# keb721/mc_water_ls_mw

Measured on AMD Instinct MI355X. Metric: mW interactions/sec/GPU (full-box + single-move ΔE), 4096-mol ice; 1/2/4/8-GPU replica scaling, higher is better.
Workload: dtype f64; 1 GPU; ih4096_t015: 4096-molecule ice-Ih boxes (8x8x8 x 8-atom cell, sigma 0.15 A), per step: full-box energy of every walker + old/new local energy of every trial move; walkers_per_gpu=512, moves_per_walker=2048, molecules=4096, parallelism=replica farm: 1 x 512 independent walkers, one process per GPU, exchange=one nccl all-reduce of 3 x 101 f64 per step (one-rank process group)

## Files before the change

### include/mw_energy.h

```cpp
#ifndef MW_ENERGY_H
#define MW_ENERGY_H

#include <stdint.h>

#ifdef __cplusplus
extern "C" {
#endif

#define MW_MAXNEIGH_LIMIT 64
#define MW_MAX_IVECT      1024

#define MW_DISPATCH_BUILD    0
#define MW_DISPATCH_ENERGY   1
#define MW_DISPATCH_MOVES    2
#define MW_DISPATCH_FORCES   3
#define MW_DISPATCH_ICE      4
#define MW_DISPATCH_RDF      5
#define MW_DISPATCH_FAMILIES 6
#define MW_DISPATCH_FIELDS   13

#define MW_LDS_ENERGY 0
#define MW_LDS_FORCES 1
#define MW_LDS_ICE    2
#define MW_LDS_MOVE   3
#define MW_LDS_SORT   4
#define MW_LDS_ORDER  5
#define MW_LDS_BUILDS 6


int mw_init(int device, int nwater, int nboxes, int maxneigh);
int mw_finalize(void);
int mw_is_initialised(void);

const char *mw_last_error(void);

int mw_constants(double out[8]);


int mw_set_cell(int ils, const double h[9], int *nivect_out);
int mw_set_cells_range(int first_ils, int count, const double *h, int *nivect_out);
int mw_get_ivects(int ils, double *out, int max_vectors, int *nivect_out);

int mw_upload_positions(int ils, const double *xyz);
int mw_download_positions(int ils, double *xyz);
int mw_upload_positions_range(int first_ils, int count, const double *xyz);
int mw_download_positions_range(int first_ils, int count, double *xyz);
int mw_patch_position(int ils, int imol, const double r[3]);


int mw_build_neighbours(int ils, int *min_nn, int *max_nn);
int mw_build_neighbours_batch(int first_ils, int count, int *min_nn, int *max_nn);
int mw_get_neighbours(int ils, int *nn, int *jn, int *vn);


int mw_model_energy(int ils, double *e);
int mw_model_energy_of(int ils, const double *xyz, double *e);
int mw_model_energy_batch(int first_ils, int count, double *e_out);
int mw_model_energy_counts(int ils, long long *npairs, long long *ntriplets);
int mw_model_energy_counts_total(int first_ils, int count, long long *npairs, long long *ntriplets);
int mw_neighbour_total(int first_ils, int count, long long *total_entries);


int mw_model_forces(int ils, double *e, double *f, double *w);
int mw_model_forces_batch(int first_ils, int count, double *e, double *f, double *w);
int mw_model_forces_launch(int first_ils, int count, int timer_slot);


int mw_ice_classes(int ils, double rc, uint8_t *cls, int counts[6]);
int mw_ice_classes_batch(int first_ils, int count, double rc, uint8_t *cls, int *counts);
int mw_ice_classes_launch(int first_ils, int count, double rc, int timer_slot);
int mw_ice_bonds(int ils, double rc, double *c);

// ... 92 lines not shown
```

### mc_water_ls_mw_amd/csrc/mw_host_ctx.hip.h

```cpp
#pragma once

namespace {

thread_local std::string g_err;
std::recursive_mutex g_mu;
std::shared_mutex g_gate;
int g_depth = 0;
struct DeviceGuard;
struct ExclusiveGuard;
#define MW_LOCK ExclusiveGuard mw_lock_; DeviceGuard mw_dev_; if (mw_lock_.rc) return 1

int fail(const char* fmt, ...)
{
    char buf[512];
    va_list ap;
    va_start(ap, fmt);
    vsnprintf(buf, sizeof buf, fmt, ap);
    va_end(ap);
    g_err = buf;
    return 1;
}

#define HIPCHK(call)                                                                             \
    do {                                                                                         \
// ... 87 lines not shown
    size_t tabscratch_n = 0;
    unsigned long long* d_wvol = nullptr;
    int* d_wflag = nullptr;
    double* d_wwin = nullptr;
    double *d_wfac = nullptr, *d_wsum = nullptr;
    int* d_winflag = nullptr;
    double* d_wmom = nullptr; size_t wmom_cap = 0;
    double* d_wstep = nullptr;
    bool has_steps = false;
    int sweep_log_ahead = 8;
    bool has_windows = false;
    int* d_wls = nullptr;
    double* d_wmu = nullptr;
    unsigned long long* d_wacc = nullptr;
    double* d_swlog = nullptr;
    size_t swlog_cap = 0;
    hipStream_t sstream = nullptr;
    mw::MailHead* h_head = nullptr;  mw::MailHead* d_head = nullptr;
    mw::MailSlot* h_slots = nullptr; mw::MailSlot* d_slots = nullptr;
    mw::MailSlot* req_slots = nullptr;
    mw::MailSlot* d_req = nullptr;
    void* req_dev_alloc = nullptr;
    int nslots = 0;
    bool srv_running = false, srv_enabled = true;
    unsigned long long sseq[8] = {0, 0, 0, 0, 0, 0, 0, 0};
    unsigned long long spend[8] = {0, 0, 0, 0, 0, 0, 0, 0};
    unsigned long long spend_epoch[8] = {0, 0, 0, 0, 0, 0, 0, 0};
    int spend_box[8] = {0, 0, 0, 0, 0, 0, 0, 0};
    hipEvent_t ev_srv = nullptr;
    double* d_pm = nullptr; int* d_srvmomok = nullptr;
    int* d_srvunc = nullptr;
    unsigned long long* d_srvcounts = nullptr;
    long long srv_starts = 0;
    int mcap = 0, mn = 0;
    int* d_mimol = nullptr;
    double *d_mtrial = nullptr, *d_meold = nullptr, *d_menew = nullptr;
    unsigned int* d_mcnt = nullptr;
    unsigned int* d_mtot = nullptr; int mtot_cap = 0, mtot_n = 0;
    int* d_mperm = nullptr;
    int* d_mdecl = nullptr;
    int mdecl_par = 0;
    int4* d_mwork = nullptr;
    int mwork_cap = 0, mwork_n = 0;
    bool mlds = false;
    int mmode = 0;
    int m_boxlo = 0, m_boxhi = -1, m_minreq = 0;
    enum { kCountsThere = 0, kCountsPending = 1, kCountsDropped = 2 };
    int mcnt_state = kCountsThere;
    int mcnt_passes = 0;
    bool move_sort = true;
    bool move_masks = true;
    bool move_gate = true;
    bool move_pairs32 = true;
    bool move_counts_eager = false;
    int move_moments = -1;
    int mchunk = 16;
    bool m_noself = false;
};

Ctx g;
std::mutex g_slot_mu[8];
std::mutex g_srv_mu;
std::atomic<unsigned long long> g_epoch{0};
std::atomic<bool> g_srv_enabled{true};

int server_stop();

struct ExclusiveGuard {
    int rc = 0;
    ExclusiveGuard()
    {
        g_mu.lock();
        if (g_depth++ == 0) {
            g_gate.lock(); g_epoch.fetch_add(1, std::memory_order_relaxed);
            g.mom_count = 0;
            if (g.srv_running) rc = server_stop();
            if (g.live && g.h_slots)
                for (int sl = 0; sl < g.nslots && sl < 8; ++sl)
                    if (g.spend[sl] && reinterpret_cast<volatile unsigned long long*>(&g.h_slots[sl].rep_seq)[0] != g.spend[sl]) {
                        reinterpret_cast<volatile unsigned long long*>(&g.h_slots[sl].rep_seq)[0] = g.spend[sl];
                        std::atomic_thread_fence(std::memory_order_seq_cst);
                    }
        }
    }
    ~ExclusiveGuard()
    {
        if (--g_depth == 0) g_gate.unlock();
        g_mu.unlock();
    }
};

struct DeviceGuard {
    int prev = -1;
    bool switched = false;
    DeviceGuard()
    {
        if (g.live && hipGetDevice(&prev) == hipSuccess && prev != g.device)
            switched = hipSetDevice(g.device) == hipSuccess;
    }
    ~DeviceGuard() { if (switched) (void)hipSetDevice(prev); }
};

constexpr size_t kQueue1024 = (size_t)(mw::kQCap + 1) * 1024 * sizeof(uint32_t);
constexpr size_t kQueue256 = (size_t)(mw::kQCap + 1) * 256 * sizeof(uint32_t);
constexpr int kFullLayout = mw::kLayoutPair;
size_t model_lds_bytes(int N, int ivcap) { return kQueue1024 + mw::lds_vec_bytes((size_t)N) + mw::lds_vec_bytes((size_t)ivcap); }
bool lds_fits(int N, int ivcap)
{
    return model_lds_bytes(N, ivcap) <= (size_t)kLdsBudget;
}
size_t pos_lds_bytes(int N, int ivcap) { return mw::lds_vec_bytes((size_t)N) + mw::lds_vec_bytes((size_t)ivcap); }
constexpr size_t kMoveScratch = 16 * sizeof(mw::WaveScratch);
size_t move_lds_bytes(int N, int ivcap, int chunk)
{
    return kMoveScratch + mw::lds_vec_bytes((size_t)ivcap) + mw::lds_vec_bytes((size_t)N) + (((size_t)N + 7) & ~(size_t)7) + (size_t)chunk * sizeof(int);
}
static_assert((size_t)kLdsBudget / 25 < ((size_t)1 << mw::kKeyMolBits), "a staged box's molecules fit the key of mw_move_energy.hip.h");
bool lds_fits_move(int N, int ivcap)
{
    return move_lds_bytes(N, ivcap, mw::kMoveChunk) <= (size_t)kLdsBudget;
}
int cell_stride(int N) { return N + 64; }
size_t sort_lds_bytes(int N) { return (size_t)N * 24 + ((size_t)cell_stride(N) + 1) * 4; }
bool sort_fits(int N) { return N <= mw::kSortBoxMax; }
void order_plan(int N, int seg_override, int& seg, int& kbits)
{
    seg = lds_fits(N, 32) ? ((N + 63) & ~63) : 64;
    if (seg_override >= 64) seg = (seg_override + 63) & ~63;
    const size_t seg_groups = ((size_t)std::min(N, seg) + 63) / 64;
    kbits = -1;
    for (int kb = 8; kb >= 0; --kb)
        if ((seg_groups << kb) <= (size_t)mw::kOrderSlots) { kbits = kb; break; }
}
size_t order_lds_bytes(int N, int seg, int kbits)
{
    return kbits < 0 ? 0 : sizeof(int) * ((((size_t)std::min(N, seg) + 63) / 64) << kbits);
}

int check_live() { return g.live ? 0 : fail("mw: engine not initialised (call mw_init / energy_init first)"); }
int check_box(int ils) { return (ils >= 1 && ils <= g.nbox) ? 0 : fail("mw: box index %d outside 1..%d", ils, g.nbox); }
int check_range(int first, int count)
{
    return (first >= 1 && count >= 1 && first + count - 1 <= g.nbox)
               ? 0 : fail("mw: box range %d..%d outside 1..%d", first, first + count - 1, g.nbox);
}
int check_mol(int imol) { return (imol >= 1 && imol <= g.N) ? 0 : fail("mw: molecule index %d outside 1..%d", imol, g.N); }
enum Form { kLaunch, kBatch, kSingle };
int check_boxes(int first, int count, Form form) { return form == kSingle ? check_box(first) : check_range(first, count); }

void drop_move_counts() { if (g.mcnt_state == Ctx::kCountsPending) g.mcnt_state = Ctx::kCountsDropped; }
void drop_driver_moments(bool state_changed = true) { g.swm_count = 0; if (state_changed) drop_move_counts(); }

int dev_free_bytes(void** p)
{
    if (!*p) return 0;
    g.owned.erase(std::remove(g.owned.begin(), g.owned.end(), *p), g.owned.end());
    void* q = *p;
    *p = nullptr;
    HIPCHK(hipFree(q));
    return 0;
}
int dev_alloc_bytes(void** p, size_t bytes)
{
    if (*p) {
        HIPCHK(hipStreamSynchronize(g.stream));
        if (dev_free_bytes(p)) return 1;
    }
    HIPCHK(hipMalloc(p, bytes));
    g.owned.push_back(*p);
// ... 67 lines not shown
```

### mc_water_ls_mw_amd/csrc/mw_host_moves.hip.h

```cpp
#pragma once

namespace {

int ensure_moves(int n)
{
    if (n <= g.mcap) return 0;
    size_t cap = 1024;
    while (cap < (size_t)n) cap *= 2;
    g.mcap = 0;
    if (dev_alloc(g.d_mimol, cap) || dev_alloc(g.d_mtrial, 3 * cap) || dev_alloc(g.d_meold, cap) || dev_alloc(g.d_menew, cap) ||
        dev_alloc(g.d_mcnt, 4 * cap) || dev_alloc(g.d_mperm, cap) || dev_alloc(g.d_mdecl, 2 * cap + 2)) return 1;
    HIPCHK(hipMemset(g.d_mdecl, 0, 2 * sizeof(int)));
    g.mdecl_par = 0;
    g.mcap = (int)cap;
    return 0;
}

template <typename Kernel>
void launch_move_kernel(Kernel kernel, size_t shmem, int kmode, const double* mom, unsigned int* tot)
{
    hipLaunchKernelGGL(kernel, dim3(g.mwork_n), dim3(1024), shmem, g.stream,
                       g.d_pos, g.d_ivect, g.d_nivect, g.d_listm, g.d_nn, g.d_mwork, g.d_mimol, g.d_mtrial, g.d_mperm,
                       g.d_meold, g.d_menew, g.d_mcnt, g.d_mdecl, g.N, g.ivcap, kmode, mom, tot);
}

}

extern "C" {

int mw_moves_upload(int n, const int* ils, const int* imol, const double* trial_xyz)
{
    MW_LOCK;
    if (check_live()) return 1;
    if (n < 0) return fail("mw_moves_upload: n = %d", n);
    drop_move_counts();
    g.mn = 0;
    if (n == 0) return 0;
    if (!ils || !imol) return fail("mw_moves_upload: null request arrays");
    std::vector<int> cnt((size_t)g.nbox + 1, 0);
    for (int m = 0; m < n; ++m) {
        if (ils[m] < 1 || ils[m] > g.nbox) return fail("mw_moves_upload: request %d has box %d outside 1..%d", m, ils[m], g.nbox);
        if (imol[m] < 1 || imol[m] > g.N) return fail("mw_moves_upload: request %d has molecule %d outside 1..%d", m, imol[m], g.N);
        ++cnt[(size_t)ils[m]];
    }
    std::vector<int> start((size_t)g.nbox + 1, 0);
    int used_boxes = 0;
    g.m_noself = true;
    g.m_boxlo = g.nbox; g.m_boxhi = -1; g.m_minreq = n;
    for (int b = 0; b < g.nbox; ++b) {
        start[(size_t)b + 1] = start[b] + cnt[(size_t)b + 1];
        if (cnt[(size_t)b + 1]) {
            ++used_boxes; if (!g.h_usegrid[(size_t)b]) g.m_noself = false;
            g.m_boxlo = std::min(g.m_boxlo, b); g.m_boxhi = std::max(g.m_boxhi, b); g.m_minreq = std::min(g.m_minreq, cnt[(size_t)b + 1]);
        }
    }
    std::vector<int> perm((size_t)n), i0((size_t)n), fill(start.begin(), start.end() - 1);
    std::vector<double> tr(trial_xyz ? (size_t)3 * n : 0);
    for (int m = 0; m < n; ++m) {
        const int s = fill[(size_t)ils[m] - 1]++;
        perm[s] = m; i0[s] = imol[m] - 1;
        if (trial_xyz) { tr[3 * (size_t)s] = trial_xyz[3 * (size_t)m]; tr[3 * (size_t)s + 1] = trial_xyz[3 * (size_t)m + 1]; tr[3 * (size_t)s + 2] = trial_xyz[3 * (size_t)m + 2]; }
    }
    g.mlds = lds_fits_move(g.N, g.ivcap) && ((long long)n * 2048 >= (long long)used_boxes * 24 * g.N);
    int chunk = 16;
    if (g.mlds) {
        const long long want = (long long)n / (2LL * std::max(1, g.cu));
        chunk = 256;
        while (chunk < mw::kMoveChunk && chunk < want) chunk *= 2;
        if (const char* ev = std::getenv("MW_MOVE_CHUNK")) { const int v = std::atoi(ev); if (v >= 64 && v <= mw::kMoveChunk) chunk = v; }
    }
    g.mchunk = chunk;
    { const char* ms = std::getenv("MW_MOVE_SORT"); g.move_sort = !(ms && ms[0] == '0'); }
    { const char* mk = std::getenv("MW_MOVE_MASKS"); g.move_masks = !(mk && mk[0] == '0'); }
    { const char* mg = std::getenv("MW_MOVE_GATE"); g.move_gate = !(mg && mg[0] == '0'); }
    { const char* mp = std::getenv("MW_MOVE_PAIRS32"); g.move_pairs32 = !(mp && mp[0] == '0'); }
    std::vector<int4> work;
    for (int b = 0; b < g.nbox; ++b) {
        const int s0 = start[b], cntb = start[(size_t)b + 1] - s0;
        if (cntb == 0) continue;
        const int nitems = (cntb + chunk - 1) / chunk;
        for (int k = 0; k < nitems; ++k) {
            int4 w; w.x = b; w.y = s0 + (int)((long long)cntb * k / nitems); w.z = s0 + (int)((long long)cntb * (k + 1) / nitems); w.w = 0;
            work.push_back(w);
        }
    }
    if (getenv("MW_NO_XCD_ORDER") == nullptr && work.size() >= 16) {
        constexpr int kXcd = 8;
        std::vector<std::vector<int4>> seq(kXcd);
        int boxrank = -1, lastbox = -1;
        for (const int4& w : work) {
            if (w.x != lastbox) { ++boxrank; lastbox = w.x; }
            seq[(size_t)(boxrank % kXcd)].push_back(w);
        }
        std::vector<int4> ordered;
        ordered.reserve(work.size());
        std::vector<size_t> at(kXcd, 0);
        while (ordered.size() < work.size())
            for (int x = 0; x < kXcd; ++x)
                if (at[x] < seq[x].size()) ordered.push_back(seq[x][at[x]++]);
        work.swap(ordered);
    }
    if (ensure_moves(n)) return 1;
    if (dev_grow(g.d_mwork, g.mwork_cap, work.size(), 2 * work.size())) return 1;
    HIPCHK(hipMemcpyAsync(g.d_mwork, work.data(), sizeof(int4) * work.size(), hipMemcpyHostToDevice, g.stream));
    HIPCHK(hipMemcpyAsync(g.d_mperm, perm.data(), sizeof(int) * n, hipMemcpyHostToDevice, g.stream));
    HIPCHK(hipMemcpyAsync(g.d_mimol, i0.data(), sizeof(int) * n, hipMemcpyHostToDevice, g.stream));
    if (trial_xyz) HIPCHK(hipMemcpyAsync(g.d_mtrial, tr.data(), sizeof(double) * 3 * n, hipMemcpyHostToDevice, g.stream));
    HIPCHK(hipStreamSynchronize(g.stream));
    g.mwork_n = (int)work.size();
    g.mn = n;
    return 0;
}

static int launch_moves(int mode)
{
    if (g.mn == 0) return 0;
    g.mcnt_state = Ctx::kCountsDropped;
    if (dev_grow(g.d_mtot, g.mtot_cap, (size_t)g.mwork_n, 2 * (size_t)g.mwork_n, 4)) return 1;
    g.mtot_n = 0;
    const size_t iv_bytes = kMoveScratch + mw::lds_vec_bytes((size_t)g.ivcap);
    const int kmode = mode | (g.mdecl_par << 2);
    g.mdecl_par ^= 1;
    const bool mom_ok = g.mlds && g.m_noself && model_geo(1).lds && g.m_boxhi >= g.m_boxlo;
    const bool fresh = g.d_mom && g.mom_count > 0 && g.mom_first - 1 <= g.m_boxlo && g.m_boxhi < g.mom_first - 1 + g.mom_count;
    const bool use_mom = mom_ok && (g.move_moments >= 0 ? g.move_moments != 0 : g.m_minreq >= (fresh ? 512 : 1280));
    const size_t shmem = g.mlds ? move_lds_bytes(g.N, g.ivcap, g.mchunk) : iv_bytes;
    auto launch = [&](auto kernel, const double* mom, unsigned int* tot, int bits = 0) { launch_move_kernel(kernel, shmem, kmode | bits, mom, tot); };
    if (use_mom) {
        if (!fresh && launch_model_energy(g.m_boxlo + 1, g.m_boxhi - g.m_boxlo + 1, true, false)) return 1;
        launch(mw::k_move_energy<true, mw::kLayoutSoA, false, true>, g.d_mom, g.d_mtot, (g.move_counts_eager ? 8 : 0) | (g.move_sort ? 32 : 0) | (g.move_masks ? 64 : 0) | (g.move_gate ? 128 : 0) | (g.move_pairs32 ? 256 : 0));
        if (g.move_counts_eager) g.mtot_n = g.mwork_n;
    } else if (g.mlds && g.m_noself) launch(mw::k_move_energy<true, mw::kLayoutSoA, false>, nullptr, nullptr);
    else if (g.mlds)                 launch(mw::k_move_energy<true>, nullptr, nullptr);
    else                             launch(mw::k_move_energy<false>, nullptr, nullptr);
    HIPCHK(hipGetLastError());
    g.mcnt_state = use_mom && !g.move_counts_eager ? Ctx::kCountsPending : Ctx::kCountsThere;
    {
        int* d = g.disp[MW_DISPATCH_MOVES];
        d[0] = g.ivcap; d[1] = g.mn; d[2] = g.mlds; d[3] = g.m_noself; d[4] = use_mom; d[5] = use_mom && fresh; d[6] = g.mchunk;
        d[7] = g.mwork_n; d[8] = (int)shmem; d[9] = use_mom ? 3 : (g.mlds ? (g.m_noself ? 2 : 1) : 0);
        d[10] = g.mcnt_state; d[11] = g.mcnt_passes; d[12] = -1;
    }
    hipLaunchKernelGGL(mw::k_move_fallback, dim3(std::min(1024, (g.mn + 3) / 4)), dim3(256), 0, g.stream, g.d_pos, g.d_ivect, g.d_listm, g.d_nn,
                       g.d_mimol, g.d_mtrial, g.d_mperm, g.d_meold, g.d_menew, g.d_mcnt, g.d_mdecl, g.N, g.ivcap, kmode);
    HIPCHK(hipGetLastError());
    g.mmode = mode;
    return 0;
}

int mw_moves_launch(void)
{
    MW_LOCK;
    if (check_live()) return 1;
    return launch_moves(3);
}

int mw_step_launch(int first_ils, int count, int timer_slot)
{
    MW_LOCK;
    if (check_live() || check_range(first_ils, count)) return 1;
    Timers t;
    if (t.open("mw_step_launch", timer_slot, 2) || t.start(0)) return 1;
    const bool want_mom = g.mn > 0 && g.mlds && g.m_noself && (g.move_moments >= 0 ? g.move_moments != 0 : g.m_minreq >= 512);
    if (launch_model_energy(first_ils, count, want_mom, true)) return 1;
    if (t.stop(0) || t.start(1) || launch_moves(3)) return 1;
    return t.stop(1);
}

int mw_moves_fetch(double* e_old, double* e_new)
{
    MW_LOCK;
    if (check_live()) return 1;
    if (g.mn > 0) {
        if (e_old) HIPCHK(hipMemcpyAsync(e_old, g.d_meold, sizeof(double) * g.mn, hipMemcpyDeviceToHost, g.stream));
        if (e_new) HIPCHK(hipMemcpyAsync(e_new, g.d_menew, sizeof(double) * g.mn, hipMemcpyDeviceToHost, g.stream));
    }
    HIPCHK(hipStreamSynchronize(g.stream));
    return 0;
}

int mw_moves_counts(long long out[4])
{
    MW_LOCK;
    if (check_live()) return 1;
    out[0] = out[1] = out[2] = out[3] = 0;
    if (g.mn == 0) return 0;
    if (g.mcnt_state == Ctx::kCountsDropped)
        return fail("mw_moves_counts: the counts of the last launch were not made, and the launch failed or the requests, positions, cells "
                    "or lists it saw have changed since: ask right after a launch (or run with MW_MOVE_COUNTS=eager)");
    if (g.mcnt_state == Ctx::kCountsPending) {
        launch_move_kernel(mw::k_move_energy<true, mw::kLayoutSoA, false, true>, move_lds_bytes(g.N, g.ivcap, g.mchunk), g.mmode | 8 | 16 | (g.move_sort ? 32 : 0) | (g.move_masks ? 64 : 0) | (g.move_gate ? 128 : 0) | (g.move_pairs32 ? 256 : 0), g.d_mom, g.d_mtot);
        HIPCHK(hipGetLastError());
        g.mtot_n = g.mwork_n;
        g.mcnt_state = Ctx::kCountsThere;
// ... 40 lines not shown
```

### mc_water_ls_mw_amd/csrc/mw_move_energy.hip.h

```cpp
#pragma once
#include <type_traits>

#include "mw_common.hip.h"
#include "mw_local_energy.hip.h"
#include "mw_move_scan.hip.h"
#include "mw_move_moments.hip.h"
#include "mw_move_lanes.hip.h"

namespace mw {

constexpr int kMoveChunk = 2048;

constexpr int kKeyMolBits = 13, kKeyReqBits = 11, kKeyNqBits = 5;
constexpr int kKeyReqShift = kKeyMolBits, kKeyNqShift = kKeyMolBits + kKeyReqBits;
constexpr uint32_t kKeyMolMask = (1u << kKeyMolBits) - 1u, kKeyReqMask = (1u << kKeyReqBits) - 1u;
constexpr int kKeyNqOver = kLaneQueue + 1;
constexpr int kSortBins = kKeyNqOver + 1;
constexpr int kSortChunks = kMoveChunk / 64;
static_assert(kMoveChunk <= (1 << kKeyReqBits) && kKeyNqOver < (1 << kKeyNqBits) && kKeyNqShift + kKeyNqBits <= 32, "the key's fields");
static_assert(kSortChunks == 2 * 16, "two rounds of the sixteen wavefronts rank an item's keys: chunks v and v + 16 in wavefront v");
static_assert((kSortChunks + 1) * kSortBins * sizeof(uint32_t) <= 16 * sizeof(WaveScratch), "the sort's tables are overlaid on the idle queues");
constexpr size_t kQueueBytes = kLaneQueueWords * sizeof(uint32_t);
constexpr size_t kMaskTableAt = 16 * kQueueBytes;
static_assert(kMaskTableAt + kMoveChunk * sizeof(uint32_t) <= 16 * sizeof(WaveScratch), "the queues and the mask table fit the scratch blocks: no new LDS");
static_assert((kSortChunks + 1) * kSortBins * sizeof(uint32_t) <= kMaskTableAt, "the sort's tables lie on the queues and end before the masks");
static_assert(kMaskTableAt % 16 == 0 && kQueueBytes % 16 == 0, "alignment of the queues and of the mask table");

template <bool LDSPOS, int LAYOUT = kLayoutSoA, bool SELFIMG = true, bool MOMPATH = false>
__global__ __launch_bounds__(1024)
void k_move_energy(const double* __restrict__ pos, const double* __restrict__ ivect,
                   const int* __restrict__ nivect, const uint32_t* __restrict__ listm,
                   const int* __restrict__ nn, const int4* __restrict__ work,
                   const int* __restrict__ req_imol, const double* __restrict__ req_trial,
                   const int* __restrict__ perm,
                   double* __restrict__ e_old, double* __restrict__ e_new,
                   unsigned int* __restrict__ counts,
                   int* __restrict__ declined,
                   int N, int ivcap, int mode, const double* __restrict__ mom = nullptr,
                   unsigned int* __restrict__ mtot = nullptr)
{
    static_assert(!MOMPATH || (LDSPOS && !SELFIMG), "the moment path serves boxes staged in LDS whose cells hold no self-images");
    __shared__ unsigned char s_qn[MOMPATH ? kCap * (kCap - 1) : 2];
    unsigned int acc[4] = {0u, 0u, 0u, 0u};
    extern __shared__ __attribute__((aligned(16))) double smem[];
    const int4 w = work[blockIdx.x];
    const int b = w.x;
    const int tid = threadIdx.x, lane = tid & 63, wave = tid >> 6;
    const bool count = !MOMPATH || (mode & 8) != 0, quiet = MOMPATH && (mode & 16) != 0;
    const double* P  = pos + (size_t)b * N * 3;
    const double* IV = ivect + (size_t)b * ivcap * 3;
    const uint32_t* LM = listm + (size_t)b * N * kRow;
    const int* NN = nn + (size_t)b * N;
    const int niv = nivect[b];

    double* spos = smem;
    double* siv = smem + (LDSPOS ? lds_vec_bytes((size_t)N) / 8 : 0);
    WaveScratch* ws = reinterpret_cast<WaveScratch*>(siv + lds_vec_bytes((size_t)ivcap) / 8) + wave;
    unsigned char* snn = reinterpret_cast<unsigned char*>(reinterpret_cast<WaveScratch*>(siv + lds_vec_bytes((size_t)ivcap) / 8) + 16);
    int* simol = reinterpret_cast<int*>(snn + (((size_t)N + 7) & ~(size_t)7));
    __shared__ int s_next;
    const int nreq = w.z - w.y;
    const double iv_first = stage_iv_begin<1024>(IV, niv, tid);
    if (LDSPOS) {
        constexpr int kB = 4;
        for (int base = 0; base < N; base += kB * 1024) {
            int v[kB];
#pragma unroll
            for (int k = 0; k < kB; ++k) { const int t = base + tid + k * 1024; v[k] = NN[t < N ? t : N - 1]; }
#pragma unroll
            for (int k = 0; k < kB; ++k) { const int t = base + tid + k * 1024; if (t < N) snn[t] = (unsigned char)v[k]; }
        }
        for (int base = 0; base < nreq; base += kB * 1024) {
            int v[kB];
#pragma unroll
            for (int k = 0; k < kB; ++k) { const int t = base + tid + k * 1024; v[k] = req_imol[w.y + (t < nreq ? t : nreq - 1)]; }
#pragma unroll
            for (int k = 0; k < kB; ++k) {
                const int t = base + tid + k * 1024;
                if (t < nreq) simol[t] = MOMPATH ? (int)((uint32_t)v[k] | (uint32_t)t << kKeyReqShift) : v[k];
            }
        }
        stage_vecs<LAYOUT, 1024>(spos, P, N, N, tid);
        if (tid == 0) s_next = 16;
    }
    stage_iv_end<LAYOUT, 1024>(siv, IV, niv, ivcap, tid, iv_first);
    __syncthreads();

    const LdsVecs<LAYOUT> vpos{spos, N}, viv{siv, ivcap};
    auto getiv = [&](int k, double& x, double& y, double& z) { viv.get(k, x, y, z); };
    auto getpos = [&](int jx, double& x, double& y, double& z) {
        if constexpr (LDSPOS) vpos.get(jx, x, y, z);
        else { const double* p = P + 3 * (size_t)jx; x = p[0]; y = p[1]; z = p[2]; }
    };
    auto row = [&](int jx, int sl) { return LM[(size_t)jx * kRow + sl]; };
    auto nnof = [&](int jx) { return LDSPOS ? (int)snn[jx] : NN[jx]; };
    auto imol_of = [&](int q) { return LDSPOS ? simol[q] : req_imol[w.y + q]; };

    auto in_lanes = [](int v) { asm volatile("" : "+v"(v)); return v; };
    auto fetch = [&](int q, int& i_, uint32_t& e_, double& t_, int& o_) {
        i_ = 0; e_ = 0u; t_ = 0.0; o_ = 0;
        if (q < nreq) {
            const int m_ = in_lanes(w.y + q);
            i_ = imol_of(q); e_ = row(i_, lane & 31);
            if (mode & 2) t_ = req_trial[3u * (unsigned)m_ + (lane < 3 ? (unsigned)lane : 0u)];
            o_ = perm[(unsigned)m_];
        }
    };
    if constexpr (MOMPATH) {
        uint32_t* wq = reinterpret_cast<uint32_t*>(ws - wave) + wave * kLaneQueueWords;
        uint32_t* smask = reinterpret_cast<uint32_t*>(ws - wave) + kMaskTableAt / sizeof(uint32_t);
        unsigned char* qn = s_qn + wave * 32;
        const double* MOM = mom + (size_t)b * N * kMomStride;
        const int rq = lane >> 1, side = lane & 1;
        uint32_t* skey = reinterpret_cast<uint32_t*>(simol);
        int nserve = nreq;
        if ((mode & 32) && nreq > 32) {
            const int ngrp_up = (nreq + 31) >> 5;
            auto image = [&](uint32_t e, double& qx, double& qy, double& qz) { lanes_image(getpos, getiv, e, qx, qy, qz); };
            auto cfetch = [&](int grp, uint32_t& k_, double (&t_)[3], uint4& c_) {
                k_ = 0u; t_[0] = t_[1] = t_[2] = 0.0; c_ = make_uint4(0u, 0u, 0u, 0u);
                const int q = grp * 32 + rq;
                if (q < nreq) {
                    const unsigned m_ = (unsigned)(w.y + q);
                    k_ = skey[q];
                    c_ = *reinterpret_cast<const uint4*>(LM + (size_t)(k_ & kKeyMolMask) * kRow);
                    if (mode & 2) { t_[0] = req_trial[3u * m_]; t_[1] = req_trial[3u * m_ + 1u]; t_[2] = req_trial[3u * m_ + 2u]; }
                }
            };
            uint32_t k; double t[3]; uint4 c4;
            cfetch(wave, k, t, c4);
            for (int grp = wave; grp < ngrp_up; grp += 16) {
                uint32_t k_nx; double t_nx[3]; uint4 c_nx;
                cfetch(grp + 16, k_nx, t_nx, c_nx);
                const int q = grp * 32 + rq;
                const int i = (int)(k & kKeyMolMask);
                double px, py, pz;
                getpos(i, px, py, pz);
                if ((mode & 2) && side) { px = t[0]; py = t[1]; pz = t[2]; }
                const int n_i = q < nreq ? min(nnof(i), kRow) : 0;
                int cnt = 0;
                bool self = false;
                uint32_t msk = 0u;
                lanes_scan<false>(image, LM + (size_t)i * kRow, wq, rq, side, i, n_i, c4, px, py, pz, cnt, self, msk);
                if (q < nreq && side == 0) {
                    skey[q] = k | (uint32_t)(self || cnt > kLaneQueue ? kKeyNqOver : cnt) << kKeyNqShift;
                    if (mode & 64) smask[q] = n_i > 32 ? kMaskScan : msk;
                }
                k = k_nx; t[0] = t_nx[0]; t[1] = t_nx[1]; t[2] = t_nx[2]; c4 = c_nx;
            }
            __syncthreads();
            uint32_t* tab = reinterpret_cast<uint32_t*>(ws - wave);
            const int nch = (nreq + 63) >> 6;
            uint32_t key[2] = {0u, 0u};
            int rank[2] = {0, 0};
#pragma unroll
            for (int h = 0; h < 2; ++h) {
                const int ch = wave + 16 * h, q = ch * 64 + lane;
                if (ch >= nch) continue;
                key[h] = q < nreq ? skey[q] : 0u;
                const int bin = q < nreq ? (int)(key[h] >> kKeyNqShift) : -1;
                unsigned int mine = 0u;
#pragma nounroll
                for (int bn = 0; bn < kSortBins; ++bn) {
                    const unsigned long long m = __ballot(bin == bn);
                    if (bin == bn) rank[h] = __popcll(m & ((1ull << lane) - 1ull));
                    if (lane == bn) mine = (unsigned int)__popcll(m);
                }
                if (lane < kSortBins) tab[ch * kSortBins + lane] = mine;
            }
            __syncthreads();
            if (wave == 0) {
                const int bin = lane <= kLaneQueue ? kLaneQueue - lane : kKeyNqOver;
                unsigned int run = 0u;
                if (lane < kSortBins) {
#pragma unroll
                    for (int ch = 0; ch < kSortChunks; ++ch)
                        if (ch < nch) { const unsigned int c = tab[ch * kSortBins + bin]; tab[ch * kSortBins + bin] = run; run += c; }
                }
                unsigned int at = 0u;
#pragma nounroll
                for (int l = 0; l + 1 < kSortBins; ++l) { const unsigned int tl = (unsigned int)__builtin_amdgcn_readlane((int)run, l); if (lane > l) at += tl; }
                if (lane < kSortBins) tab[kSortChunks * kSortBins + bin] = at;
            }
            __syncthreads();
#pragma unroll
            for (int h = 0; h < 2; ++h) {
                const int ch = wave + 16 * h;
                if (ch * 64 + lane < nreq) {
                    const int bin = (int)(key[h] >> kKeyNqShift);
                    skey[tab[kSortChunks * kSortBins + bin] + tab[ch * kSortBins + bin] + (unsigned int)rank[h]] = key[h];
                }
            }
            nserve = __builtin_amdgcn_readfirstlane((int)tab[kSortChunks * kSortBins + kKeyNqOver]);
            __syncthreads();
            if (!quiet)
                for (int p = nserve + tid; p < nreq; p += 1024) {
                    const int k2 = atomicAdd(&declined[(mode >> 2) & 1], 1);
                    declined[2 + 2 * k2] = w.y + (int)((skey[p] >> kKeyReqShift) & kKeyReqMask); declined[3 + 2 * k2] = b;
                }
        }
        const int ngrp = (nserve + 31) >> 5;
        const bool masks = (mode & 64) && (mode & 32) && nreq > 32;
        auto fetch = [&](int grp, uint32_t& k_, int& o_, double (&t_)[3], uint32_t (&e_)[kLaneWalk], bool& walk_) {
            k_ = 0u; o_ = 0; t_[0] = t_[1] = t_[2] = 0.0; walk_ = false;
#pragma unroll
            for (int c = 0; c < kLaneWalk; ++c) e_[c] = 0u;
            if (grp < ngrp) {
                k_ = skey[min(grp * 32 + rq, nserve - 1)];
                const unsigned m_ = (unsigned)w.y + ((k_ >> kKeyReqShift) & kKeyReqMask);
                const unsigned at = (k_ & kKeyMolMask) * (unsigned)kRow;
                if (masks) {
                    const uint32_t msk = grp * 32 + rq < nserve ? smask[(k_ >> kKeyReqShift) & kKeyReqMask] : 0u;
                    walk_ = __ballot(msk == kMaskScan) == 0ull;
                    if (walk_) lanes_entries(LM, at, msk, side, e_);
                }
                if (!walk_) {
                    const uint4 c_ = *reinterpret_cast<const uint4*>(LM + at);
                    e_[0] = c_.x; e_[1] = c_.y; e_[2] = c_.z; e_[3] = c_.w;
                }
                if (mode & 2) { t_[0] = req_trial[3u * m_]; t_[1] = req_trial[3u * m_ + 1u]; t_[2] = req_trial[3u * m_ + 2u]; }
                o_ = perm[m_];
            }
        };
        int cur = wave;
        uint32_t k; int o; double t[3]; uint32_t e8[kLaneWalk]; bool walk;
        fetch(cur, k, o, t, e8, walk);
        while (cur < ngrp) {
            int nxt = 0;
            if (lane == 0) nxt = __hip_atomic_fetch_add(&s_next, 1, __ATOMIC_RELAXED, __HIP_MEMORY_SCOPE_WORKGROUP);
            nxt = __builtin_amdgcn_readfirstlane(nxt);
            uint32_t k_nx; int o_nx; double t_nx[3]; uint32_t e_nx[kLaneWalk]; bool walk_nx;
            const bool valid = cur * 32 + rq < nserve;
            const int i = (int)(k & kKeyMolMask);
            double px, py, pz;
            getpos(i, px, py, pz);
            if ((mode & 2) && side) { px = t[0]; py = t[1]; pz = t[2]; }
            const int n_i = valid ? min(nnof(i), kRow) : 0;
            double en = 0.0;
            unsigned int ci = 0u, cs = 0u;
            const bool served = move_energy_mom_lanes(getpos, getiv, nnof, LM + (size_t)i * kRow, MOM, wq, qn, i, n_i,
                                                      walk, valid ? (int)(k >> kKeyNqShift) : 0, e8,
                                                      px, py, pz, lane, count, (mode & 128) != 0, (mode & 256) != 0, en, ci, cs);
            fetch(nxt, k_nx, o_nx, t_nx, e_nx, walk_nx);
            if (valid && !served) {
                if (side == 0 && !quiet) {
                    const int k = atomicAdd(&declined[(mode >> 2) & 1], 1);
                    declined[2 + 2 * k] = w.y + (int)((skey[cur * 32 + rq] >> kKeyReqShift) & kKeyReqMask); declined[3 + 2 * k] = b;
                }
            } else if (valid) {
                const size_t so = (size_t)o;
                if (side == 0 && (mode & 1)) { if (!quiet) e_old[so] = en; if (count) { counts[4 * so] = 0u; counts[4 * so + 1] = 0u; } }
                if (side == 1 && (mode & 2)) { if (!quiet) e_new[so] = en; if (count) { counts[4 * so + 2] = 0u; counts[4 * so + 3] = 0u; } }
                if (count) { acc[0] += ci; acc[1] += cs; }
            }
            wave_fence();
            cur = nxt; k = k_nx; o = o_nx; t[0] = t_nx[0]; t[1] = t_nx[1]; t[2] = t_nx[2]; walk = walk_nx;
#pragma unroll
            for (int c = 0; c < kLaneWalk; ++c) e8[c] = e_nx[c];
        }
    } else {
        int cur = wave;
        int i, o; uint32_t e; double t;
        fetch(cur, i, e, t, o);
        while (cur < nreq) {
            int nxt = 0;
            if (lane == 0) nxt = __hip_atomic_fetch_add(&s_next, 1, __ATOMIC_RELAXED, __HIP_MEMORY_SCOPE_WORKGROUP);
            nxt = LDSPOS ? __builtin_amdgcn_readfirstlane(nxt) : nreq;
            int i_nx, o_nx; uint32_t e_nx; double t_nx;
            fetch(nxt, i_nx, e_nx, t_nx, o_nx);

            const int m = w.y + cur;
            double xo, yo, zo;
            getpos(i, xo, yo, zo);
            double xn = xo, yn = yo, zn = zo;
            if (mode & 2) { xn = readlane_f64(t, 0); yn = readlane_f64(t, 1); zn = readlane_f64(t, 2); }

            MoveRes r;
            const bool fast = move_energy_wave<SELFIMG>(getpos, getiv, row, nnof, ws, niv, i, nnof(i), e, xo, yo, zo, xn, yn, zn, lane, r);
            asm volatile("" : "+v"(e_nx), "+v"(t_nx), "+v"(o_nx));
            if (!fast) {
                if (lane == 0 && !quiet) {
                    const int k = atomicAdd(&declined[(mode >> 2) & 1], 1);
                    declined[2 + 2 * k] = m; declined[3 + 2 * k] = b;
                }
            } else if (lane == 0) {
                const size_t so = (size_t)o;
                if (mode & 1) { if (!quiet) e_old[so] = r.eo; if (count) { counts[4 * so] = r.io; counts[4 * so + 1] = r.so; } }
                if (mode & 2) { if (!quiet) e_new[so] = r.en; if (count) { counts[4 * so + 2] = r.in_; counts[4 * so + 3] = r.sn; } }
            }
            cur = nxt; i = i_nx; e = e_nx; t = t_nx; o = o_nx;
        }
    }
    if constexpr (MOMPATH) if (count) {
        if (lane & 1) { acc[2] = acc[0]; acc[3] = acc[1]; acc[0] = acc[1] = 0u; }
    }
    if constexpr (MOMPATH) if (count) {
        __shared__ unsigned int s_tot[16][4];
#pragma unroll
        for (int c = 0; c < 4; ++c) {
            const int tot = dpp_wave_sum_i32((int)acc[c]);
            if (lane == 63) s_tot[wave][c] = (unsigned int)tot;
        }
        __syncthreads();
        if (tid < 4) {
            unsigned int t = 0u;
            for (int wv = 0; wv < 16; ++wv) t += s_tot[wv][tid];
            mtot[4 * (size_t)blockIdx.x + tid] = t;
        }
    }
}

__global__ __launch_bounds__(256)
void k_move_fallback(const double* __restrict__ pos, const double* __restrict__ ivect,
                     const uint32_t* __restrict__ listm, const int* __restrict__ nn,
                     const int* __restrict__ req_imol, const double* __restrict__ req_trial, const int* __restrict__ perm,
                     double* __restrict__ e_old, double* __restrict__ e_new, unsigned int* __restrict__ counts,
                     int* __restrict__ declined, int N, int ivcap, int mode)
{
    const int par = (mode >> 2) & 1;
    const int n = declined[par];
    if (blockIdx.x == 0 && threadIdx.x == 0) declined[par ^ 1] = 0;
    const int lane = threadIdx.x & 63;
    const int wave = (int)(blockIdx.x * (blockDim.x >> 6)) + (int)(threadIdx.x >> 6), nwaves = (int)(gridDim.x * (blockDim.x >> 6));
    for (int k = wave; k < 2 * n; k += nwaves) {
        const int side = k & 1;
        if (!((mode >> side) & 1)) continue;
        const int m = declined[2 + 2 * (k >> 1)], b = declined[3 + 2 * (k >> 1)];
        const double* P  = pos + (size_t)b * N * 3;
        const double* IV = ivect + (size_t)b * ivcap * 3;
        const uint32_t* LM = listm + (size_t)b * N * kRow;
        const int* NN = nn + (size_t)b * N;
        const int i = req_imol[m];
        const size_t o = (size_t)perm[m];
        Override none; none.idx = -1; none.x = none.y = none.z = 0.0;
        Override tr; tr.idx = -1; tr.x = tr.y = tr.z = 0.0;
        if (side) { tr.idx = i; tr.x = req_trial[3 * (size_t)m]; tr.y = req_trial[3 * (size_t)m + 1]; tr.z = req_trial[3 * (size_t)m + 2]; }
        unsigned int ni, ns;
        const double en = local_energy_wave_batched<false>(P, IV, LM, NN, i, tr, none, lane, ni, ns);
        if (lane == 0) {
            (side ? e_new : e_old)[o] = en;
            counts[4 * o + 2 * side] = ni; counts[4 * o + 2 * side + 1] = ns;
        }
    }
}

__global__ __launch_bounds__(64)
void k_local_energy_single(double* __restrict__ pos, const double* __restrict__ ivect,
                           const uint32_t* __restrict__ listm, const int* __restrict__ nn,
                           int b, int i, Override o1, Override o2, int commit,
                           double* __restrict__ e_out, int N, int ivcap,
                           unsigned long long* __restrict__ done, unsigned long long seq)
{
    const int lane = threadIdx.x;
    double* P = pos + (size_t)b * N * 3;
    unsigned int ni, ns;
    const double e = local_energy_wave(P, ivect + (size_t)b * ivcap * 3, listm + (size_t)b * N * kRow,
                                       nn + (size_t)b * N, i, o1, o2, lane, ni, ns);
    if (lane == 0) {
        *e_out = e;
        if (commit) {
// ... 12 lines not shown
```

### mc_water_ls_mw_amd/energy.py

```python
from __future__ import annotations

import ctypes
import os
import sys

import numpy as np

PKG = os.path.dirname(os.path.abspath(__file__))
LIB_PATH = os.path.join(PKG, "libmw_hip.so")
MAXNEIGH = 50

_dp = ctypes.POINTER(ctypes.c_double)
_ip = ctypes.POINTER(ctypes.c_int)
_llp = ctypes.POINTER(ctypes.c_longlong)
_fp = ctypes.POINTER(ctypes.c_float)

ABI_SYMBOLS = (
    "mw_init", "mw_finalize", "mw_is_initialised", "mw_last_error", "mw_constants",
    "mw_set_cell", "mw_get_ivects", "mw_upload_positions", "mw_download_positions", "mw_patch_position",
    "mw_upload_positions_range", "mw_download_positions_range", "mw_set_cells_range",
    "mw_build_neighbours", "mw_build_neighbours_batch", "mw_get_neighbours",
    "mw_model_energy", "mw_model_energy_of", "mw_model_energy_batch", "mw_model_energy_counts",
    "mw_model_energy_counts_total", "mw_neighbour_total",
    "mw_model_forces", "mw_model_forces_batch", "mw_model_forces_launch",
    "mw_ice_classes", "mw_ice_classes_batch", "mw_ice_classes_launch", "mw_ice_bonds",
    "mw_ice_clusters", "mw_ice_clusters_batch", "mw_ice_clusters_launch", "mw_ice_clusters_plan", "mw_ice_clusters_last",
    "mw_rdf", "mw_rdf_batch", "mw_rdf_launch",
    "mw_local_energy", "mw_local_energy_patched", "mw_local_energy_post", "mw_local_energy_collect",
    "mw_server_counts", "mw_local_energy_batch", "mw_delta_energy_batch",
    "mw_moves_upload", "mw_moves_launch", "mw_moves_fetch", "mw_moves_counts",
    "mw_model_energy_launch", "mw_step_launch", "mw_model_energy_fetch", "mw_build_neighbours_launch", "mw_sync",
    "mw_timer_start", "mw_timer_stop", "mw_timer_elapsed_ms", "mw_device_info",
    "mw_sweep_configure", "mw_set_model_energy", "mw_sweep_set_state", "mw_sweep_set_states_range", "mw_sweep_get_state",
    "mw_sweep_translation", "mw_sweep_translation_launch", "mw_sweep_lds_bytes", "mw_sweep_last_launch",
    "mw_sweep_options", "mw_sweep_get_tables", "mw_sweep_set_tables", "mw_sweep_get_switches", "mw_sweep_get_shifts_range",
    "mw_sweep_reduce_tables", "mw_sweep_broadcast_tables",
    "mw_sweep_get_tables_range", "mw_sweep_set_tables_range",
    "mw_sweep_moves", "mw_sweep_get_volume_moves", "mw_sweep_sync_cells", "mw_sweep_check_flags",
    "mw_sweep_leshift", "mw_sweep_minu", "mw_sweep_swetnam", "mw_sweep_dd", "mw_sweep_windows", "mw_sweep_set_factors", "mw_sweep_get_factors", "mw_sweep_steps", "mw_sweep_get_counters",
    "mw_last_dispatch", "mw_lds_plan",
)

DISPATCH_FIELDS = {
    "build": ("ivcap", "boxes", "grid_boxes", "brute_boxes", "fused_sort", "legacy_search", "order_seg", "nseg", "lds_bytes"),
    "energy": ("ivcap", "boxes", "lds", "nsplit", "chunk", "grid_y", "moments", "lds_bytes", "block"),
    "moves": ("ivcap", "requests", "mlds", "noself", "use_mom", "fresh", "mchunk", "items", "lds_bytes", "build", "counts", "count_passes", "declined"),
    "forces": ("ivcap", "boxes", "lds", "nsplit", "lds_bytes"),
    "ice": ("ivcap", "boxes", "lds", "nsplit", "lds_bytes"),
    "rdf": ("ivcap", "boxes", "small", "workgroups_per_box", "lds_bytes", "images"),
}
LDS_BUILDS = ("energy", "forces", "ice", "move", "sort", "order")


def lds_plan(nwater, image_capacity=32):
    L = load_library()
    out = (ctypes.c_int * (2 * len(LDS_BUILDS)))()
    if L.mw_lds_plan(int(nwater), int(image_capacity), out, len(out)) != len(LDS_BUILDS):
        raise MwError(f"mw_lds_plan: no plan for {nwater} molecules, {image_capacity} image vectors")
    return {b: (bool(out[2 * k]), int(out[2 * k + 1])) for k, b in enumerate(LDS_BUILDS)}


class MwError(RuntimeError):
    """A C-ABI call returned nonzero; the text is mw_last_error()."""


_lib = None


def load_library(path=LIB_PATH):
    global _lib
    if _lib is not None:
        return _lib
    path = os.environ.get("MW_HIP_LIB", path)
    if not os.path.exists(path):
        raise MwError(f"{path} not found: build it with `python -m mc_water_ls_mw_amd.build` "
                      "(the mW engine has no CPU fallback)")
    _share_hip_runtime_with_torch()
    L = ctypes.CDLL(path)
    L.mw_last_error.restype = ctypes.c_char_p
    _lib = L
    return L


def _share_hip_runtime_with_torch():
    if "torch" in sys.modules:
        return
    try:
        import importlib.util
        spec = importlib.util.find_spec("torch")
    except (ImportError, ValueError):
        spec = None
    if spec is None or not spec.origin:
        return
    cand = os.path.join(os.path.dirname(spec.origin), "lib", "libamdhip64.so")
    if os.path.exists(cand):
        try:
            ctypes.CDLL(cand, mode=ctypes.RTLD_GLOBAL)
        except OSError:
            pass


def _d(a):
    return a.ctypes.data_as(_dp)
# ... 557 lines not shown
```

Baseline: 496.6 billion interactions/s.

## Make moment-path move kernel persistent with prefetched next-item staging

The moment-path move energy kernel now launches at most one workgroup per CU and loops over work items. While it finishes the current item, it prefetches the next item's request keys and, when the box changes, the box's neighbour counts, positions and image vectors into registers before writing them to LDS. This is meant to cut workgroup launch and LDS restaging overhead and to overlap global loads with the tail of the previous item. It also changes the per-request counts written in the masked path and adds dispatch fields plus environment knobs. The trade-offs are register pressure and serialized items within a CU.

```diff
diff --git a/include/mw_energy.h b/include/mw_energy.h
--- a/include/mw_energy.h
+++ b/include/mw_energy.h
@@ -17,7 +17,7 @@
 #define MW_DISPATCH_ICE      4
 #define MW_DISPATCH_RDF      5
 #define MW_DISPATCH_FAMILIES 6
-#define MW_DISPATCH_FIELDS   13
+#define MW_DISPATCH_FIELDS   15
 
 #define MW_LDS_ENERGY 0
 #define MW_LDS_FORCES 1
diff --git a/mc_water_ls_mw_amd/csrc/mw_host_ctx.hip.h b/mc_water_ls_mw_amd/csrc/mw_host_ctx.hip.h
--- a/mc_water_ls_mw_amd/csrc/mw_host_ctx.hip.h
+++ b/mc_water_ls_mw_amd/csrc/mw_host_ctx.hip.h
@@ -163,6 +163,8 @@
     bool move_masks = true;
     bool move_gate = true;
     bool move_pairs32 = true;
+    bool move_persist = true;
+    int move_persist_wgs = 0;
     bool move_counts_eager = false;
     int move_moments = -1;
     int mchunk = 16;
@@ -226,6 +228,11 @@
 {
     return kMoveScratch + mw::lds_vec_bytes((size_t)ivcap) + mw::lds_vec_bytes((size_t)N) + (((size_t)N + 7) & ~(size_t)7) + (size_t)chunk * sizeof(int);
 }
+int move_grid(int items)
+{
+    if (g.move_persist_wgs > 0) return std::min(items, g.move_persist_wgs);
+    return g.move_persist && items > g.cu && g.cu > 0 ? g.cu : items;
+}
 static_assert((size_t)kLdsBudget / 25 < ((size_t)1 << mw::kKeyMolBits), "a staged box's molecules fit the key of mw_move_energy.hip.h");
 bool lds_fits_move(int N, int ivcap)
 {
diff --git a/mc_water_ls_mw_amd/csrc/mw_host_moves.hip.h b/mc_water_ls_mw_amd/csrc/mw_host_moves.hip.h
--- a/mc_water_ls_mw_amd/csrc/mw_host_moves.hip.h
+++ b/mc_water_ls_mw_amd/csrc/mw_host_moves.hip.h
@@ -19,9 +19,9 @@
 template <typename Kernel>
 void launch_move_kernel(Kernel kernel, size_t shmem, int kmode, const double* mom, unsigned int* tot)
 {
-    hipLaunchKernelGGL(kernel, dim3(g.mwork_n), dim3(1024), shmem, g.stream,
+    hipLaunchKernelGGL(kernel, dim3(mom ? move_grid(g.mwork_n) : g.mwork_n), dim3(1024), shmem, g.stream,
                        g.d_pos, g.d_ivect, g.d_nivect, g.d_listm, g.d_nn, g.d_mwork, g.d_mimol, g.d_mtrial, g.d_mperm,
-                       g.d_meold, g.d_menew, g.d_mcnt, g.d_mdecl, g.N, g.ivcap, kmode, mom, tot);
+                       g.d_meold, g.d_menew, g.d_mcnt, g.d_mdecl, g.N, g.ivcap, kmode, mom, tot, g.mwork_n);
 }
 
 }
@@ -74,6 +74,8 @@
     { const char* mk = std::getenv("MW_MOVE_MASKS"); g.move_masks = !(mk && mk[0] == '0'); }
     { const char* mg = std::getenv("MW_MOVE_GATE"); g.move_gate = !(mg && mg[0] == '0'); }
     { const char* mp = std::getenv("MW_MOVE_PAIRS32"); g.move_pairs32 = !(mp && mp[0] == '0'); }
+    { const char* pe = std::getenv("MW_MOVE_PERSIST"); g.move_persist = !(pe && pe[0] == '0'); }
+    { const char* pw = std::getenv("MW_MOVE_PERSIST_WGS"); g.move_persist_wgs = pw ? std::max(0, std::atoi(pw)) : 0; }
     std::vector<int4> work;
     for (int b = 0; b < g.nbox; ++b) {
         const int s0 = start[b], cntb = start[(size_t)b + 1] - s0;
@@ -140,6 +142,7 @@
         d[0] = g.ivcap; d[1] = g.mn; d[2] = g.mlds; d[3] = g.m_noself; d[4] = use_mom; d[5] = use_mom && fresh; d[6] = g.mchunk;
         d[7] = g.mwork_n; d[8] = (int)shmem; d[9] = use_mom ? 3 : (g.mlds ? (g.m_noself ? 2 : 1) : 0);
         d[10] = g.mcnt_state; d[11] = g.mcnt_passes; d[12] = -1;
+        d[13] = use_mom ? move_grid(g.mwork_n) : g.mwork_n; d[14] = use_mom && g.move_persist;
     }
     hipLaunchKernelGGL(mw::k_move_fallback, dim3(std::min(1024, (g.mn + 3) / 4)), dim3(256), 0, g.stream, g.d_pos, g.d_ivect, g.d_listm, g.d_nn,
                        g.d_mimol, g.d_mtrial, g.d_mperm, g.d_meold, g.d_menew, g.d_mcnt, g.d_mdecl, g.N, g.ivcap, kmode);
diff --git a/mc_water_ls_mw_amd/csrc/mw_move_energy.hip.h b/mc_water_ls_mw_amd/csrc/mw_move_energy.hip.h
--- a/mc_water_ls_mw_amd/csrc/mw_move_energy.hip.h
+++ b/mc_water_ls_mw_amd/csrc/mw_move_energy.hip.h
@@ -26,6 +26,20 @@
 static_assert((kSortChunks + 1) * kSortBins * sizeof(uint32_t) <= kMaskTableAt, "the sort's tables lie on the queues and end before the masks");
 static_assert(kMaskTableAt % 16 == 0 && kQueueBytes % 16 == 0, "alignment of the queues and of the mask table");
 
+constexpr int kStageBatch = 12;
+template <int THREADS>
+__device__ __forceinline__ void stage_vecs_load(double (&v)[kStageBatch], const double* __restrict__ src, int total, int base, int tid)
+{
+#pragma unroll
+    for (int k = 0; k < kStageBatch; ++k) { const int t = base + tid + k * THREADS; v[k] = src[t < total ? t : total - 1]; }
+}
+template <int LAYOUT, int THREADS>
+__device__ __forceinline__ void stage_vecs_store(double* __restrict__ dst, const double (&v)[kStageBatch], int total, int n, int base, int tid)
+{
+#pragma unroll
+    for (int k = 0; k < kStageBatch; ++k) { const int t = base + tid + k * THREADS; if (t < total) dst[LdsVecs<LAYOUT>::slot(t, n)] = v[k]; }
+}
+
 template <bool LDSPOS, int LAYOUT = kLayoutSoA, bool SELFIMG = true, bool MOMPATH = false>
 __global__ __launch_bounds__(1024)
 void k_move_energy(const double* __restrict__ pos, const double* __restrict__ ivect,
@@ -37,14 +51,15 @@
                    unsigned int* __restrict__ counts,
                    int* __restrict__ declined,
                    int N, int ivcap, int mode, const double* __restrict__ mom = nullptr,
-                   unsigned int* __restrict__ mtot = nullptr)
+                   unsigned int* __restrict__ mtot = nullptr,
+                   int nitems = 0)
 {
     static_assert(!MOMPATH || (LDSPOS && !SELFIMG), "the moment path serves boxes staged in LDS whose cells hold no self-images");
     __shared__ unsigned char s_qn[MOMPATH ? kCap * (kCap - 1) : 2];
     unsigned int acc[4] = {0u, 0u, 0u, 0u};
     extern __shared__ __attribute__((aligned(16))) double smem[];
-    const int4 w = work[blockIdx.x];
-    const int b = w.x;
+    int4 w = work[blockIdx.x];
+    int b = w.x;
     const int tid = threadIdx.x, lane = tid & 63, wave = tid >> 6;
     const bool count = !MOMPATH || (mode & 8) != 0, quiet = MOMPATH && (mode & 16) != 0;
     const double* P  = pos + (size_t)b * N * 3;
@@ -59,7 +74,7 @@
     unsigned char* snn = reinterpret_cast<unsigned char*>(reinterpret_cast<WaveScratch*>(siv + lds_vec_bytes((size_t)ivcap) / 8) + 16);
     int* simol = reinterpret_cast<int*>(snn + (((size_t)N + 7) & ~(size_t)7));
     __shared__ int s_next;
-    const int nreq = w.z - w.y;
+    int nreq = w.z - w.y;
     const double iv_first = stage_iv_begin<1024>(IV, niv, tid);
     if (LDSPOS) {
         constexpr int kB = 4;
@@ -107,12 +122,18 @@
         }
     };
     if constexpr (MOMPATH) {
-        uint32_t* wq = reinterpret_cast<uint32_t*>(ws - wave) + wave * kLaneQueueWords;
-        uint32_t* smask = reinterpret_cast<uint32_t*>(ws - wave) + kMaskTableAt / sizeof(uint32_t);
+        uint32_t* const scr = reinterpret_cast<uint32_t*>(ws - wave);
+        uint32_t* smask = scr + kMaskTableAt / sizeof(uint32_t);
+        uint32_t* skey = reinterpret_cast<uint32_t*>(simol);
+        const int wave_s = __builtin_amdgcn_readfirstlane(wave);
+        for (int item = blockIdx.x;;) {
+        int lane0 = 0;
+        asm volatile("" : "+s"(lane0));
+        const int wave = wave_s, lane = (int)__builtin_amdgcn_mbcnt_hi(~0u, __builtin_amdgcn_mbcnt_lo(~0u, (unsigned)lane0)), tid = wave * 64 + lane;
+        uint32_t* wq = scr + wave * kLaneQueueWords;
         unsigned char* qn = s_qn + wave * 32;
+        const int rq = lane >> 1, side = lane & 1;
         const double* MOM = mom + (size_t)b * N * kMomStride;
-        const int rq = lane >> 1, side = lane & 1;
-        uint32_t* skey = reinterpret_cast<uint32_t*>(simol);
         int nserve = nreq;
         if ((mode & 32) && nreq > 32) {
             const int ngrp_up = (nreq + 31) >> 5;
@@ -149,7 +170,7 @@
                 k = k_nx; t[0] = t_nx[0]; t[1] = t_nx[1]; t[2] = t_nx[2]; c4 = c_nx;
             }
             __syncthreads();
-            uint32_t* tab = reinterpret_cast<uint32_t*>(ws - wave);
+            uint32_t* tab = scr;
             const int nch = (nreq + 63) >> 6;
             uint32_t key[2] = {0u, 0u};
             int rank[2] = {0, 0};
@@ -249,14 +270,72 @@
                 }
             } else if (valid) {
                 const size_t so = (size_t)o;
-                if (side == 0 && (mode & 1)) { if (!quiet) e_old[so] = en; if (count) { counts[4 * so] = 0u; counts[4 * so + 1] = 0u; } }
-                if (side == 1 && (mode & 2)) { if (!quiet) e_new[so] = en; if (count) { counts[4 * so + 2] = 0u; counts[4 * so + 3] = 0u; } }
+                if (side == 0 && (mode & 1)) { if (!quiet) e_old[so] = en; if (count) { counts[4 * so] = (unsigned)in_lanes(0); counts[4 * so + 1] = (unsigned)in_lanes(0); } }
+                if (side == 1 && (mode & 2)) { if (!quiet) e_new[so] = en; if (count) { counts[4 * so + 2] = (unsigned)in_lanes(0); counts[4 * so + 3] = (unsigned)in_lanes(0); } }
                 if (count) { acc[0] += ci; acc[1] += cs; }
             }
             wave_fence();
             cur = nxt; k = k_nx; o = o_nx; t[0] = t_nx[0]; t[1] = t_nx[1]; t[2] = t_nx[2]; walk = walk_nx;
 #pragma unroll
             for (int c = 0; c < kLaneWalk; ++c) e8[c] = e_nx[c];
+        }
+        const int item_nx = item + (int)gridDim.x;
+        const bool more = item_nx < nitems;
+        constexpr int kB = 4;
+        const int4 w_nx = work[more ? item_nx : item];
+        const bool newbox = w_nx.x != b;
+        const int nreq_nx = w_nx.z - w_nx.y;
+        const int* NNn = nn + (size_t)w_nx.x * N;
+        const double* IVn = ivect + (size_t)w_nx.x * ivcap * 3;
+        const double* Pn = pos + (size_t)w_nx.x * N * 3;
+        int nn_nx[kB] = {}, key_nx[kB] = {}, niv_nx = 0;
+        double pos_nx[kStageBatch] = {}, iv_nx = 0.0;
+        if (more) {
+#pragma unroll
+            for (int c = 0; c < kB; ++c) { const int q = tid + c * 1024; key_nx[c] = req_imol[w_nx.y + (q < nreq_nx ? q : nreq_nx - 1)]; }
+            if (newbox) {
+#pragma unroll
+                for (int c = 0; c < kB; ++c) { const int q = tid + c * 1024; nn_nx[c] = NNn[q < N ? q : N - 1]; }
+                niv_nx = nivect[w_nx.x];
+                iv_nx = stage_iv_begin<1024>(IVn, niv_nx, tid);
+                stage_vecs_load<1024>(pos_nx, Pn, 3 * N, 0, tid);
+            }
+        }
+        __shared__ unsigned int s_tot[16][4];
+        if (count) {
+            if (lane & 1) { acc[2] = acc[0]; acc[3] = acc[1]; acc[0] = acc[1] = 0u; }
+#pragma unroll
+            for (int c = 0; c < 4; ++c) {
+                const int tot = dpp_wave_sum_i32((int)acc[c]);
+                if (lane == 63) s_tot[wave][c] = (unsigned int)tot;
+            }
+        }
+        if (count || more) __syncthreads();
+        if (count && tid < 4) {
+            unsigned int t = 0u;
+            for (int wv = 0; wv < 16; ++wv) t += s_tot[wv][tid];
+            mtot[4 * (size_t)item + tid] = t;
+        }
+        if (!more) break;
+#pragma unroll
+        for (int c = 0; c < kB; ++c) { const int q = tid + c * 1024; if (q < nreq_nx) skey[q] = (uint32_t)key_nx[c] | (uint32_t)q << kKeyReqShift; }
+        if (newbox) {
+            b = w_nx.x;
+            LM = listm + (size_t)b * N * kRow;
+#pragma unroll
+            for (int c = 0; c < kB; ++c) { const int q = tid + c * 1024; if (q < N) snn[q] = (unsigned char)nn_nx[c]; }
+            for (int q = tid + kB * 1024; q < N; q += 1024) snn[q] = (unsigned char)NNn[q];
+            stage_vecs_store<LAYOUT, 1024>(spos, pos_nx, 3 * N, N, 0, tid);
+            for (int base = kStageBatch * 1024; base < 3 * N; base += kStageBatch * 1024) {
+                stage_vecs_load<1024>(pos_nx, Pn, 3 * N, base, tid);
+                stage_vecs_store<LAYOUT, 1024>(spos, pos_nx, 3 * N, N, base, tid);
+            }
+            stage_iv_end<LAYOUT, 1024>(siv, IVn, niv_nx, ivcap, tid, iv_nx);
+        }
+        if (tid == 0) s_next = 16;
+        w = w_nx; nreq = nreq_nx; item = item_nx;
+        acc[0] = acc[1] = acc[2] = acc[3] = 0u;
+        __syncthreads();
         }
     } else {
         int cur = wave;
@@ -289,23 +368,6 @@
                 if (mode & 2) { if (!quiet) e_new[so] = r.en; if (count) { counts[4 * so + 2] = r.in_; counts[4 * so + 3] = r.sn; } }
             }
             cur = nxt; i = i_nx; e = e_nx; t = t_nx; o = o_nx;
-        }
-    }
-    if constexpr (MOMPATH) if (count) {
-        if (lane & 1) { acc[2] = acc[0]; acc[3] = acc[1]; acc[0] = acc[1] = 0u; }
-    }
-    if constexpr (MOMPATH) if (count) {
-        __shared__ unsigned int s_tot[16][4];
-#pragma unroll
-        for (int c = 0; c < 4; ++c) {
-            const int tot = dpp_wave_sum_i32((int)acc[c]);
-            if (lane == 63) s_tot[wave][c] = (unsigned int)tot;
-        }
-        __syncthreads();
-        if (tid < 4) {
-            unsigned int t = 0u;
-            for (int wv = 0; wv < 16; ++wv) t += s_tot[wv][tid];
-            mtot[4 * (size_t)blockIdx.x + tid] = t;
         }
     }
 }
diff --git a/mc_water_ls_mw_amd/energy.py b/mc_water_ls_mw_amd/energy.py
--- a/mc_water_ls_mw_amd/energy.py
+++ b/mc_water_ls_mw_amd/energy.py
@@ -2,6 +2,7 @@
 
 import ctypes
 import os
+import re
 import sys
 
 import numpy as np
@@ -44,11 +45,28 @@
 DISPATCH_FIELDS = {
     "build": ("ivcap", "boxes", "grid_boxes", "brute_boxes", "fused_sort", "legacy_search", "order_seg", "nseg", "lds_bytes"),
     "energy": ("ivcap", "boxes", "lds", "nsplit", "chunk", "grid_y", "moments", "lds_bytes", "block"),
-    "moves": ("ivcap", "requests", "mlds", "noself", "use_mom", "fresh", "mchunk", "items", "lds_bytes", "build", "counts", "count_passes", "declined"),
+    "moves": ("ivcap", "requests", "mlds", "noself", "use_mom", "fresh", "mchunk", "items", "lds_bytes", "build", "counts", "count_passes", "declined",
+              "grid", "persist"),
     "forces": ("ivcap", "boxes", "lds", "nsplit", "lds_bytes"),
     "ice": ("ivcap", "boxes", "lds", "nsplit", "lds_bytes"),
     "rdf": ("ivcap", "boxes", "small", "workgroups_per_box", "lds_bytes", "images"),
 }
+
+
+def move_grid(items, compute_units, env=None):
+    env = os.environ if env is None else env
+
+    def atoi(text):
+        m = re.match(r"\s*([+-]?\d+)", text)
+        return int(m.group(1)) if m else 0
+
+    forced = max(0, atoi(env["MW_MOVE_PERSIST_WGS"])) if "MW_MOVE_PERSIST_WGS" in env else 0
+    if forced > 0:
+        return min(items, forced)
+    persist = not env.get("MW_MOVE_PERSIST", "").startswith("0")
+    return compute_units if persist and items > compute_units > 0 else items
+
+
 LDS_BUILDS = ("energy", "forces", "ice", "move", "sort", "order")
 
 
```

After: 492.9 billion interactions/s (median of 2 runs). About the same (-0.7%).
